# alexandrainst/coral

Hardware: AMD Instinct MI355X
Metric: audio-seconds/sec (CTC finetune step: fwd+bwd+allreduce+clip+AdamW), wav2vec2-large, 10 s utterances (higher is better)
Workload: dtype bf16; 1 GPU; wav2vec2-large (XLS-R shape d=1920 L=48 ffn=7680) CTC finetune, 8 x 10 s per GPU, SpecAugment on, activation_dropout 0.1, layerdrop 0 (multi-GPU rule), fp32 master + AdamW + clip 1.0; global_batch=8, frames_per_utt=499, parallelism=dp1

## Files before the change

### coral_amd/_lib.py

```python

from __future__ import annotations

import ctypes as C
import os
from pathlib import Path

_HERE = Path(__file__).resolve().parent
LIB_PATH = _HERE / "libcoral_amd.so"


class CoralAmdError(RuntimeError):
    """Raised when the HIP library is missing or a call into it fails."""


class CaGemmDesc(C.Structure):

    _fields_ = [
        ("A", C.c_void_p),
        ("B", C.c_void_p),
        ("C", C.c_void_p),
        ("C2", C.c_void_p),
        ("R", C.c_void_p),
        ("bias", C.c_void_p),
        ("M", C.c_int32),
# ... 202 lines not shown
    "ca_wave_normalize": (C.c_int, [_vp, _vp, _vp, _i32, _i64, _f32, _vp]),
    "ca_frame_lengths": (C.c_int, [_vp, _i32, _i64, C.POINTER(C.c_int32), C.POINTER(C.c_int32), _i32, _vp, _vp]),
    "ca_wave_scale": (C.c_int, [_vp, _vp, _vp, _i32, _i64, _vp]),
    "ca_fir_filter": (C.c_int, [_vp, _vp, _vp, _vp, _vp, _i64, _i32, _vp, _i32, _i64, _vp]),
    "ca_mix_noise": (C.c_int, [_vp, _vp, _vp, _i64, _i64, _vp, _vp, _vp, _vp, _i32, _i64, _vp]),
    "ca_white_noise": (C.c_int, [_vp, _i64, C.c_uint64, _vp]),
    "ca_pcm_prepare": (C.c_int, [_vp, _i32, _i64, _vp, _vp, _vp, _i32, _i64, _i32, _i32, _f32, _vp]),
    "ca_resample": (C.c_int, [_vp, _i32, _i64, _vp, _vp, _i32, _vp, _vp, _i32, _i32, _i32, _vp, _i64, _vp, _i32, _vp]),
    "ca_conv0_ln_gelu_fwd": (
        C.c_int,
        [_vp, _vp, _vp, _vp, _vp, _vp, _i32, _i64, _i32, _i32, _i32, _f32, _vp],
    ),
    "ca_conv0_bwd_partial_floats": (_i64, [_i32, _i64, _i32, _i32, _i32]),
    "ca_conv0_ln_gelu_bwd": (
        C.c_int,
        [_vp] * 11 + [_i32, _i64, _i32, _i32, _i32, _f32, _vp],
    ),
    "ca_col2im_1d": (C.c_int, [_vp, _vp, _i32, _i64, _i64, _i32, _i32, _i32, _vp]),
    "ca_ctc_workspace_bytes": (_i64, [_i32, _i32, _i32]),
    "ca_ctc_loss_fwd_bwd": (
        C.c_int,
        [_vp, _vp, _vp, _vp, _vp, _vp, _vp, _i32, _i32, _i32, _i64, _i32, _i32, _i32, _vp],
    ),
    "ca_ctc_greedy_decode": (
        C.c_int,
        [_vp, _vp, _vp, _vp, _vp, _i32, _i32, _i32, _i64, _i32, _vp],
    ),
    "ca_ctc_stitch": (C.c_int, [_vp, _vp, _vp, _vp, _i32, _i32, _i32, _i64, _i32, _i32, _vp]),
    "ca_ctc_collapse_workspace_bytes": (_i64, [_i32, _i32]),
    "ca_ctc_collapse_offsets": (C.c_int, [_vp, _vp, _vp, _vp, _vp, _vp, _vp, _i64, _i32, _i32, _i32, _vp]),
    "ca_ctc_beam_workspace_bytes": (_i64, [_i32, _i32, _i32, _i32]),
    "ca_ctc_beam_decode": (C.c_int, [C.POINTER(CaCtcBeamDesc), _vp]),
    "ca_ctc_align_workspace_bytes": (_i64, [_i32, _i32, _i32]),
    "ca_ctc_align": (C.c_int, [_vp, _i64, _vp, _vp, _vp, _vp, _vp, _vp, _vp, _vp, _i64, _i32, _i32, _i32, _i32, _i32,
                               _vp]),
    "ca_edit_counts_workspace_bytes": (_i64, [_i32, _i64, _i64]),
    "ca_edit_counts": (C.c_int, [_vp, _vp, _vp, _vp, _vp, _i32, _vp, _i32, _vp, _i64, _vp]),
    "ca_beam_select_workspace_bytes": (_i64, [_i32, _i32, _i32]),
    "ca_beam_select": (C.c_int, [_vp, _i64, _vp, _vp, _i32, _i32, _i32, _vp, _vp, _vp, _vp, _i64, _vp]),
    "ca_beam_advance": (C.c_int, [C.POINTER(CaBeamDesc), _vp]),
    "ca_mask_frames": (C.c_int, [_vp, _vp, _vp, _vp, _vp, _i32, _i32, _i32, _vp]),
    "ca_regroup_pad": (C.c_int, [_vp, _vp, _i32, _i32, _i32, _i32, _i32, _vp]),
    "ca_posconv_partial_floats": (_i64, [_i32]),
    "ca_posconv_weight": (C.c_int, [_vp, _vp, _vp, _vp, _vp, _vp, _i32, _i32, _i32, _vp]),
    "ca_posconv_weight_bwd": (
        C.c_int,
# ... 96 lines not shown
```

### coral_amd/blocks.py

```python

from __future__ import annotations

import os

import torch

from . import ops
from .ops import EPI_DGELU, EPI_GELU, EPI_RESIDUAL, MNMAJOR


LN_IN_GEMM = os.environ.get("CA_DECODE_LN_FUSED", "1") != "0"


def _z(n, dev, dt=torch.bfloat16):
    return torch.zeros(n, dtype=dt, device=dev)


def zeros_on(dev):
    return lambda n, dt=torch.bfloat16: _z(n, dev, dt)


class Scratch:

    def __init__(self, M, d, f, z, Mkv=0, masks=True):
# ... 268 lines not shown
        if defer is None:
            ops.colsum(sc.du, f, M, f, g32, sc.part, out_off=o(self.fc1 + ".bias"))
        wg.append(dict(dY=sc.du, X=sv["x"], M=f, N=d, K=M, lda=f, ldb=d, c_off=o(self.fc1 + ".weight"), accumulate=acc,
                       sq=sq.get("fc1"),
                       **(dict(bias_off=o(self.fc1 + ".bias"), part=sc.part, cs_off=self.cs_fc1) if defer is not None else {})))
        if defer is not None:
            defer.extend(wg)
        else:
            ops.wgrad_gemm_group(wg, g32)
        if du8 is not None and du8["ready"][0]:
            ops.gemm_fp8(du8["buf"], fb[0], sc.dx, a_scale=du8["inv"], b_scale=du8["inv_w"], M=M, N=d, K=f, lda=f, ldb=f, ldc=d,
                         b_off=du8["w_off"])
        else:
            ops.gemm(sc.du, p16, sc.dx, M=M, N=d, K=f, lda=f, b_layout=MNMAJOR, ldb=d, ldc=d, b_off=o(self.fc1 + ".weight"))
        _ln_bwd(st, self.ln, sc.dx, sv, dh, dhin, sc, M, d, ln_part, pending, xdrop)


def wgrad_stream(engine):
    if os.environ.get("CA_WGRAD_STREAM", "1") == "0":
        return None
    if engine._wstream is None:
        engine._wstream = ops.side_stream(engine.device, "wgrad", int(os.environ.get("CA_WGRAD_PRIO", "0")))
    return engine._wstream


def norm_plan(store, matrices, device):
    if not matrices:
        return None
    off, soff, mats = 0, {}, []
    for l, key, name, M, N in matrices:
        soff[(l, key)] = off
        off += ops.sumsq_slots(M, N)
        mats.append((store.off(name), M * N))
    chunks, pos = [], 0
    for a, n in sorted(mats) + [(store.numel, 0)]:
        while pos < a:
            m = min(65536, a - pos)
            chunks.append((pos, m))
            pos += m
        pos = max(pos, a + n)
    return dict(slots=torch.zeros(off, dtype=torch.float32, device=device), nslots=off, slot_off=soff,
                chunks=torch.tensor(chunks, dtype=torch.int64, device=device), nchunks=len(chunks),
                partial=torch.zeros(max(4096, len(chunks)), dtype=torch.float32, device=device))


def encoder_backward(blocks, svs, keep, B, T, ring, scs, bias_ws, ln_parts, *, gm, acc, plan, names, side, wgrad_early,
                     matrix_range, done, below=None, mring=None, epilogue=None, rows=None):
    main = torch.cuda.current_stream()
    M = B * T if rows is None else rows[1]
    kw_rows = {} if rows is None else dict(rows=rows)

    def on_side(fn):
        if side is None:
            return fn()
        ev = torch.cuda.Event()
        ev.record(main)
        side.wait_event(ev)
        with torch.cuda.stream(side):
            return fn()

    wdone, it = {}, 0
    for l in reversed(range(len(blocks))):
        if not keep[l]:
            if not acc:
                lo, hi = matrix_range(l)
                ops.clear_ranges(gm, ((lo, hi - lo),))
                if plan is not None:
                    a0 = plan["slot_off"][(l, "qkv")]
                    ops.clear_f32(plan["slots"], plan["slot_off"].get((l + 1, "qkv"), plan["nslots"]) - a0, off=a0)
            done(names[l])
# ... 16 lines not shown

        def wgrads():
            fused[0] = ops.wgrad_gemm_group(wg, gm, colsum_ws=bw, colsum_ld=nb, Gb=g32)

        ff.backward(ring[i0], ring[i1], sv_f, sc, M, defer=wg, acc=acc, sq=sq, ln_part=lnp[0], pending=second, **kw_f)
        sa.backward(ring[i1], ring[i2], sv_a, sc, B, T, defer=wg, acc=acc, sq=sq, ln_part=lnp[1], pending=second,
                    deferred=(lambda: on_side(wgrads)) if wgrad_early else None, **kw_a, **kw_rows)

        def finish():
            if not wgrad_early:
                wgrads()
            if fused[0]:
                second.append((bw, ops.COLSUM_PARTS, nb, nb, g32[st.off(sa.qbias):], True))
            ops.reduce_rows_multi(second)
            if epilogue is not None:
                epilogue(l)
            if side is not None:
                wdone[it] = torch.cuda.Event()
                wdone[it].record(side)
            done(names[l])

        on_side(finish)
        it += 1
    if side is not None:
        main.wait_stream(side)
    k = (2 * it) % 6
    return ring[k], (mring[k] if mring is not None else None), ring[(k + 1) % 6]
```

### coral_amd/csrc/ctc.hip

```cpp
#include "common.h"

#define NEG_INF (-__builtin_inff())

__device__ __forceinline__ float log_add3(float a, float b, float c) {
  const float m = fmaxf(a, fmaxf(b, c));
  if (m == NEG_INF) return NEG_INF;
  return m + __logf(__expf(a - m) + __expf(b - m) + __expf(c - m));
}
__device__ __forceinline__ float log_add2(float a, float b) {
  const float m = fmaxf(a, b);
  if (m == NEG_INF) return NEG_INF;
  return m + __logf(__expf(a - m) + __expf(b - m));
}

struct CtcWs {
  float* lp;
  float* alpha;
  float* beta;
};

__device__ __host__ inline int64_t align256(int64_t x) { return (x + 255) & ~(int64_t)255; }

extern "C" int64_t ca_ctc_workspace_bytes(int32_t B, int32_t T, int32_t Lmax) {
  const int64_t S = 2 * (int64_t)Lmax + 1;
// ... 197 lines not shown
    }
  }
  if (tid == 0) {
    float nll;
    if (Tin <= 0) {
      nll = __builtin_inff();
    } else {
      const int lastrow = (Tin - 1) & 1;
      const float l1 = rowa[lastrow][S - 1];
      const float l2 = S >= 2 ? rowa[lastrow][S - 2] : NEG_INF;
      nll = -log_add2(l1, l2);
    }
    sh_nll = nll;
  }
  __syncthreads();
  float nll = sh_nll;
  const bool infeasible = !(nll < __builtin_inff());
  if (tid == 0) {
    nll_out[b] = (infeasible && zero_inf) ? 0.f : nll;
    raw_nll[b] = nll;
  }
}

__global__ __launch_bounds__(512) void ctc_grad_kernel(const int32_t* __restrict__ labels,
                                                       const int32_t* __restrict__ in_len,
                                                       const float* __restrict__ raw_nll, float* __restrict__ grad,
                                                       const float* __restrict__ gscale, const float* __restrict__ lp,
                                                       const float* __restrict__ alpha, const float* __restrict__ beta,
                                                       int T, int V, int64_t ldv, int Lmax, int Smax, int blank) {
  __shared__ int ext[CTC_MAXS];
  __shared__ float vm[8][256], vs[8][256];
  __shared__ int sh_L;
  const int b = blockIdx.y;
  const int tid = threadIdx.x;
  const int lane = tid & 63, wave = tid >> 6;
  if (tid == 0) {
    int L = 0;
    for (int i = 0; i < Lmax; ++i) {
      const int c = labels[(int64_t)b * Lmax + i];
      if (c >= 0) {
        ext[2 * L] = blank;
        ext[2 * L + 1] = c;
        ++L;
      }
    }
    ext[2 * L] = blank;
    sh_L = L;
  }
  __syncthreads();
  const int S = 2 * sh_L + 1;
  int Tin = in_len ? in_len[b] : T;
  if (Tin > T) Tin = T;
  if (Tin < 0) Tin = 0;
  const float nll = raw_nll[b];
  const bool infeasible = !(nll < __builtin_inff());
  const float gs = gscale ? gscale[b] : 1.f;
  const int t = blockIdx.x * 8 + wave;
  if (t >= T) return;
  float* g = grad + ((int64_t)b * T + t) * ldv;
  if (t >= Tin || infeasible) {
    for (int v = lane; v < (int)ldv; v += 64) g[v] = 0.f;
    return;
  }
  float* vmax = vm[wave];
  float* vsum = vs[wave];
  for (int v = lane; v < V; v += 64) {
    vmax[v] = NEG_INF;
    vsum[v] = 0.f;
  }
  const float* at = alpha + ((int64_t)b * T + t) * Smax;
// ... 33 lines not shown
  CA_CHECK_ARG(B > 0 && T > 0 && V > 0 && V <= 256 && ldv >= V && Lmax >= 0,
               "ca_ctc_loss_fwd_bwd: bad shape (V must be <= 256)");
  CA_CHECK_ARG(2 * Lmax + 1 <= CTC_MAXS, "ca_ctc_loss_fwd_bwd: Lmax %d too long (max %d)", Lmax,
               (CTC_MAXS - 1) / 2);
  CA_CHECK_ARG(blank >= 0 && blank < V, "ca_ctc_loss_fwd_bwd: bad blank");
  const int Smax = 2 * Lmax + 1;
  char* w = (char*)ws;
  float* lp = (float*)w;
  w += align256((int64_t)B * T * 256 * 4);
  float* alpha = (float*)w;
  w += align256((int64_t)B * T * Smax * 4);
  float* beta = (float*)w;
  w += align256((int64_t)B * T * Smax * 4);
  float* raw_nll = (float*)w;
  hipStream_t s = (hipStream_t)stream;
  const int64_t frames = (int64_t)B * T;
  hipLaunchKernelGGL(ctc_logsoftmax_kernel, dim3((unsigned)((frames + 3) / 4)), dim3(256), 0, s, logits, lp, frames, V,
                     ldv);
  const size_t lp_bytes = (size_t)T * V * sizeof(float);
  const int lp_in_lds = lp_bytes <= 120 * 1024 ? 1 : 0;
  static bool attr = false;
  if (!attr) {
    hipFuncSetAttribute((const void*)ctc_kernel, hipFuncAttributeMaxDynamicSharedMemorySize, 120 * 1024);
    attr = true;
  }
  hipLaunchKernelGGL(ctc_kernel, dim3(B), dim3(512), lp_in_lds ? lp_bytes : 0, s, labels, in_len, nll, raw_nll, lp, alpha,
                     beta, T, V, Lmax, Smax, blank, zero_infinity, lp_in_lds);
  if (grad)
    hipLaunchKernelGGL(ctc_grad_kernel, dim3((unsigned)((T + 7) / 8), B), dim3(512), 0, s, labels, in_len, raw_nll, grad,
                       gscale, lp, alpha, beta, T, V, ldv, Lmax, Smax, blank);
  CA_CHECK_LAUNCH("ca_ctc_loss_fwd_bwd");
  return CA_OK;
}

__global__ __launch_bounds__(1024) void ctc_greedy_kernel(const float* __restrict__ logits,
                                                          const int32_t* __restrict__ in_len,
                                                          int32_t* __restrict__ raw,
                                                          int32_t* __restrict__ ids,
                                                          int32_t* __restrict__ out_len, int T,
                                                          int V, int64_t ldv, int blank) {
  extern __shared__ int sh[];
  const int b = blockIdx.x;
  const float* lg = logits + (int64_t)b * T * ldv;
  int32_t* rb = raw + (int64_t)b * T;
  int32_t* ib = ids + (int64_t)b * T;
  int Tin = in_len ? in_len[b] : T;
  if (Tin > T) Tin = T;
  for (int t = threadIdx.x; t < T; t += 1024) {
    const float* l = lg + (int64_t)t * ldv;
    float best = l[0];
// ... 46 lines not shown
```

### coral_amd/stem_blocks.py

```python

from __future__ import annotations

import torch

from . import ops
from .blocks import layernorm_bwd
from .ops import EPI_GELU_RESIDUAL, EPI_RESIDUAL, MNMAJOR

F32 = torch.float32


class ConvScratch:

    def __init__(self, z, B, wgrad, dgrad, part):
        nw = max(c.Co * c.k * c.Ci for c in wgrad)
        self.dwr_part, self.dwr = z(B * nw, F32), z(nw, F32)
        self.dcol = z(max(B * c.T * c.k * c.Ci for c in dgrad))
        self.part = part


class StridedConvBlock:

    def __init__(self, store, weight: str, bias: str, Ci: int, Co: int, k: int, stride: int, rows_in=None, rows_out=None,
                 y_off: int = 0):
        self.st, self.Ci, self.Co, self.k, self.stride, self.y_off = store, Ci, Co, k, stride, y_off
        self.w_off, self.b_off = store.off(weight), store.off(bias)
        self.wr = torch.zeros(Co * k * Ci, dtype=torch.bfloat16, device=store.device)
        if rows_in is not None:
            self.set_rows(rows_in, rows_out)

    def set_rows(self, rows_in: int, rows_out=None):
        self.rows_in = rows_in
        self.T = (rows_in - self.k) // self.stride + 1
        self.rows_out = self.T if rows_out is None else rows_out
        assert self.y_off + self.T <= self.rows_out

    def refresh(self):
        ops.conv_weight_reorder(self.st.p32, self.wr, self.Co, self.Ci, self.k, w_off=self.w_off)

    def forward(self, x, y, B, **epilogue):
        Ci, Co, k = self.Ci, self.Co, self.k
        ops.gemm(x, self.wr, y, c_off=self.y_off * Co, M=self.T, N=Co, K=k * Ci, lda=self.stride * Ci, ldb=k * Ci, ldc=Co,
                 bias=self.st.p32, bias_off=self.b_off, batch2=B, sA=(0, self.rows_in * Ci), sC=(0, self.rows_out * Co),
                 **epilogue)

    def backward(self, dy, x, B, sc: ConvScratch, dx=None):
        Ci, Co, k, T = self.Ci, self.Co, self.k, self.T
        g32, nw = self.st.g32, Co * k * Ci
        clips, rows = (1, B * T) if self.rows_out == T else (B, T)
        for b in range(clips):
            ops.colsum(dy, Co, rows, Co, g32, sc.part, x_off=(b * self.rows_out + self.y_off) * Co, out_off=self.b_off)
        ops.gemm(dy, x, sc.dwr_part, M=Co, N=k * Ci, K=T, a_layout=MNMAJOR, lda=Co, a_off=self.y_off * Co, b_layout=MNMAJOR,
                 ldb=self.stride * Ci, ldc=k * Ci, out_f32=True, batch2=B, sA=(0, self.rows_out * Co),
                 sB=(0, self.rows_in * Ci), sC=(0, nw))
        ops.reduce_rows(sc.dwr_part, B, nw, nw, sc.dwr)
        ops.conv_weight_grad_reorder(sc.dwr, g32, Co, Ci, k, dw_off=self.w_off)
        if dx is not None:
            assert self.rows_out == T, "the data gradient reads dy as one [B * T, Co] matrix"
            ops.gemm(dy, self.wr, sc.dcol, M=B * T, N=k * Ci, K=Co, lda=Co, b_layout=MNMAJOR, ldb=k * Ci, ldc=k * Ci)
            ops.col2im_1d(sc.dcol, dx, B, T, self.rows_in, Ci, k, self.stride)


class ConvFeatureEncoder:

    def __init__(self, store, prefix: str, conv_dim, conv_kernel, conv_stride, eps: float, f32: bool):
        assert conv_dim[0] == 512 and conv_kernel[0] == 10, "layer-0 kernel expects C=512,k=10"
        self.st, self.eps, self.f32 = store, eps, f32
        self.dims, self.k0, self.stride0 = tuple(conv_dim), conv_kernel[0], conv_stride[0]
        names = [[f"{prefix}{i}.{n}" for n in ("conv.weight", "conv.bias", "layer_norm.weight", "layer_norm.bias")]
                 for i in range(len(conv_dim))]
        self.p = [[store.view(n) for n in ns] for ns in names]
        self.g = [[store.view(n, "g32") for n in ns] for ns in names]
        self.convs = [None] + [StridedConvBlock(store, names[i][0], names[i][1], conv_dim[i - 1], conv_dim[i], conv_kernel[i],
                                                conv_stride[i]) for i in range(1, len(conv_dim))]

    def refresh(self):
        for c in self.convs[1:]:
            c.refresh()

    def alloc(self, B, Ts, z, part):
        n = [B * T * C for T, C in zip(Ts, self.dims)]
        bf, cdt = torch.bfloat16, F32 if self.f32 else torch.bfloat16
        for i, c in enumerate(self.convs[1:], 1):
            c.set_rows(Ts[i - 1])
        return dict(Ts=Ts, a=[z(m, dt=bf) for m in n[:-1]] + [z(n[-1], dt=cdt)], y=[None] + [z(m, dt=cdt) for m in n[1:]],
                    cstats=[None] + [z(B * T * 2, dt=F32) for T in Ts[1:]], dconv=[z(m) for m in n], dy=z(max(n[1:])),
                    sc=ConvScratch(z, B, self.convs[1:], self.convs[1:], part))

    def forward(self, x, sv, B, N):
        a, y, Ts = sv["a"], sv["y"], sv["Ts"]
        ops.conv0_fwd(x, *self.p[0], a[0], B, N, self.dims[0], self.k0, self.stride0, self.eps)
        for i, c in enumerate(self.convs[1:], 1):
            c.set_rows(Ts[i - 1])
            c.forward(a[i - 1], y[i], B)
            ops.layernorm_fwd(y[i], self.p[i][2], self.p[i][3], a[i], sv["cstats"][i], B * Ts[i], c.Co, self.eps, act=1)
        return a[-1]

    def backward(self, x, sv, B, N):
        dconv, dy, sc, Ts = sv["dconv"], sv["dy"], sv["sc"], sv["Ts"]
        for i in range(len(self.convs) - 1, 0, -1):
            c, (_, _, gamma, beta), (_, _, dgamma, dbeta) = self.convs[i], self.p[i], self.g[i]
            ops.layernorm_bwd(dconv[i], sv["y"][i], gamma, beta, sv["cstats"][i], None, dy, dgamma, dbeta, sc.part,
                              B * Ts[i], c.Co, act=1)
            c.backward(dy, sv["a"][i - 1], B, sc, dx=dconv[i - 1])
        ops.conv0_bwd(x, *self.p[0], dconv[0], *self.g[0], sc.part, B, N, self.dims[0], self.k0, self.stride0, self.eps)


class FeatureProjection:

    def __init__(self, store, prefix: str, C: int, d: int, eps: float):
        self.st, self.C, self.d, self.eps = store, C, d, eps
        ln = prefix + "layer_norm."
        self.gamma, self.beta = store.view(ln + "weight"), store.view(ln + "bias")
        self.dgamma, self.dbeta = store.view(ln + "weight", "g32"), store.view(ln + "bias", "g32")
        self.w_off, self.b_off = store.off(prefix + "projection.weight"), store.off(prefix + "projection.bias")

    def alloc(self, M, z):
        return dict(xln=z(M * self.C), st=z(M * 2, dt=F32))

    def forward(self, x, h0, sv, M, drop=(0.0, 0)):
        st, C, d = self.st, self.C, self.d
        ops.layernorm_fwd(x, self.gamma, self.beta, sv["xln"], sv["st"], M, C, self.eps)
        ops.gemm(sv["xln"], st.p16, h0, M=M, N=d, K=C, lda=C, ldb=C, ldc=d, b_off=self.w_off, bias=st.p32, bias_off=self.b_off)
        if drop[0] > 0:
            ops.dropout(h0, h0, M * d, *drop)

    def backward(self, dh0, x, dxln, dx, sv, M, part, drop=(0.0, 0)):
        st, C, d = self.st, self.C, self.d
        if drop[0] > 0:
            ops.dropout(dh0, dh0, M * d, *drop)
        ops.colsum(dh0, d, M, d, st.g32, part, out_off=self.b_off)
        ops.gemm(dh0, sv["xln"], st.g32, M=d, N=C, K=M, a_layout=MNMAJOR, lda=d, b_layout=MNMAJOR, ldb=C, ldc=C,
                 c_off=self.w_off, out_f32=True, accumulate=True)
        ops.gemm(dh0, st.p16, dxln, M=M, N=C, K=d, lda=d, b_layout=MNMAJOR, ldb=C, ldc=C, b_off=self.w_off)
        ops.layernorm_bwd(dxln, x, self.gamma, None, sv["st"], None, dx, self.dgamma, self.dbeta, part, M, C)


class PosConvEmbed:

    def __init__(self, store, prefix: str, d: int, G: int, K: int):
        self.st, self.d, self.G, self.K, self.Cg = store, d, G, K, d // G
        dev = store.device
        self.wf = torch.zeros(d * K * self.Cg, dtype=torch.bfloat16, device=dev)
        self.wb = torch.zeros(d * K * self.Cg, dtype=torch.bfloat16, device=dev)
        self.norm = torch.zeros(K, dtype=F32, device=dev)
        self.partial = torch.zeros(ops.posconv_partial_floats(K), dtype=F32, device=dev)
        w = prefix + "parametrizations.weight."
        self.v, self.g = store.view(w + "original1"), store.view(w + "original0")
        self.dv, self.dg = store.view(w + "original1", "g32"), store.view(w + "original0", "g32")
        self.b_off = store.off(prefix + "bias")

    def refresh(self):
        ops.posconv_weight(self.v, self.g, self.wf, self.wb, self.norm, self.partial, self.d, self.Cg, self.K)

    def alloc(self, B, T, z):
        n = B * self.G * (T + self.K) * self.Cg + 8 * self.Cg
        return dict(xg=z(n), pc_pre=z(B * T * self.d), dxg=z(n), dwf=z(self.d * self.K * self.Cg, dt=F32))

    def _conv(self, T, Tpad):
        G, K, Cg, d = self.G, self.K, self.Cg, self.d
        return dict(M=T, N=Cg, K=K * Cg, lda=Cg, ldb=K * Cg, ldc=d, ldr=d, batch2=G, sA=(G * Tpad * Cg, Tpad * Cg),
                    sB=(0, Cg * K * Cg), sC=(T * d, Cg), sR=(T * d, Cg))

    def forward(self, h0, h, sv, B, T):
        st, G, K, Cg = self.st, self.G, self.K, self.Cg
        ops.regroup_pad(h0, sv["xg"], B, T, G, Cg, K // 2)
        ops.gemm(sv["xg"], self.wf, sv["pc_pre"], C2=h, R=h0, bias=st.p32, bias_off=self.b_off, epilogue=EPI_GELU_RESIDUAL,
                 batch1=B, sBias=(0, Cg), **self._conv(T, T + K))

    def backward(self, dh, dpc, dh0, sv, B, T, part):
        st, d, G, K, Cg = self.st, self.d, self.G, self.K, self.Cg
        M, Tpad = B * T, T + K
        ops.dgelu_mul(dh, sv["pc_pre"], dpc, M * d)
        ops.colsum(dpc, d, M, d, st.g32, part, out_off=self.b_off)
        ops.gemm(dpc, sv["xg"], sv["dwf"], M=Cg, N=K * Cg, K=M, a_layout=MNMAJOR, lda=d, b_layout=MNMAJOR, ldb=Cg, b_kseg=T,
                 b_kseg_stride=G * Tpad * Cg, ldc=K * Cg, batch2=G, sA=(0, Cg), sB=(0, Tpad * Cg), sC=(0, Cg * K * Cg),
                 out_f32=True)
        ops.posconv_weight_bwd(sv["dwf"], self.v, self.g, self.norm, self.dv, self.dg, self.partial, d, Cg, K)
        ops.regroup_pad(dpc, sv["dxg"], B, T, G, Cg, K // 2)
        ops.gemm(sv["dxg"], self.wb, dh0, a_off=Cg, epilogue=EPI_RESIDUAL, R=dh, batch1=B, **self._conv(T, Tpad))


class LMHead:

    def __init__(self, store, ln: str, weight: str, bias: str | None, d: int, V: int, eps: float):
        self.st, self.d, self.V, self.Vp, self.eps = store, d, V, (V + 7) // 8 * 8, eps
        self.gamma, self.beta = store.view(ln + ".weight"), store.view(ln + ".bias")
        self.dgamma, self.dbeta = store.view(ln + ".weight", "g32"), store.view(ln + ".bias", "g32")
        self.w_off = store.off(weight)
        self.b_off = store.off(bias) if bias is not None else None

    def alloc(self, M, z, train=True):
        return dict(hf=z(M * self.d), st=z(M * 2, dt=F32) if train else None)

    def forward(self, h, sv, M, logits=None, last_of=None, drop=(0.0, 0)):
        d, hf = self.d, sv["hf"]
        ops.layernorm_fwd(h, self.gamma, self.beta, hf, sv["st"], M, d, self.eps)
        if drop[0] > 0:
            ops.dropout(hf, hf, M * d, *drop)
        if last_of is None:
            return self.project(hf, M, logits)
# ... 23 lines not shown
```

### coral_amd/wav2vec2.py

```python

from __future__ import annotations

import math
import os
from dataclasses import dataclass

import torch

from . import ops
from .blocks import FFNBlock, Scratch, SelfAttnBlock, encoder_backward, wgrad_stream
from .engine import Engine
from .staging import PinnedStager
from .stem_blocks import ConvFeatureEncoder, FeatureProjection, LMHead, PosConvEmbed


@dataclass
class Wav2Vec2Shape:

    hidden_size: int = 1024
    num_hidden_layers: int = 24
    num_attention_heads: int = 16
    intermediate_size: int = 4096
    conv_dim: tuple = (512,) * 7
    conv_kernel: tuple = (10, 3, 3, 3, 3, 2, 2)
    conv_stride: tuple = (5, 2, 2, 2, 2, 2, 2)
    num_conv_pos_embeddings: int = 128
    num_conv_pos_embedding_groups: int = 16
    vocab_size: int = 46
    pad_token_id: int = 45
    layer_norm_eps: float = 1e-5
    ctc_loss_reduction: str = "sum"
    ctc_zero_infinity: bool = True
    activation_dropout: float = 0.0
# ... 314 lines not shown
        for k, st in zip(self.s.conv_kernel, self.s.conv_stride):
            n = torch.div(n - k, st, rounding_mode="floor") + 1
        return n

    def _workspace(self, B: int, N: int):
        key = (B, N)
        if self._ws_key == key:
            return self._ws
        s, dev = self.s, self.device
        d, f = s.hidden_size, s.intermediate_size
        L = s.num_hidden_layers
        Ts = self.conv_lengths(N)
        T = Ts[-1]
        M = B * T
        bf, f32 = torch.bfloat16, torch.float32

        def build(z):
            w = {"B": B, "N": N, "Ts": Ts, "T": T, "M": M}
            pf = max(
                ops.layernorm_bwd_partial_floats(B * Ts[1], 512), ops.layernorm_bwd_partial_floats(M, d),
                ops.colsum_partial_floats(M, max(f, 3 * d)), ops.colsum_partial_floats(B * Ts[1], 512),
                ops.conv0_bwd_partial_floats(B, N, s.conv_dim[0], s.conv_kernel[0], s.conv_stride[0]), 4096)
            w["partial"] = z(pf, dt=f32)
            w["fe"] = self.feature_encoder.alloc(B, Ts, z, w["partial"])
            w["fp"] = self.feature_projection.alloc(M, z)
            w["h0"] = z(M * d)
            w["pc"] = self.pos_conv.alloc(B, T, z)
            w["h"] = [z(M * d) for _ in range(L + 1)]
            w["hpk"] = z(M * d)
            w["h1"] = [z(M * d) for _ in range(L)]
            w["sv"] = [(sa.alloc(B, T, z), ff.alloc(M, z)) for sa, ff in self.blocks]
            w["head"] = self.head.alloc(M, z)
            Vp = w["Vp"] = self.head.Vp
            w["logits"] = z(M * Vp, dt=f32)
            w["dlogits"] = z(M * Vp, dt=f32)
            w["dlogits16"] = z(M * Vp)
            w["dlogits16p"] = z(M * Vp)
            w["nll"] = z(B, dt=f32)
            w["dA"] = z(M * d)
            w["ring"] = [z(M * d) for _ in range(6)]
            w["mring"] = [z(M * d) for _ in range(6)] if s.hidden_dropout > 0 else None
            w["scs"] = [Scratch(M, d, f, z, masks=False) for _ in range(2)]
            w["bias_ws"] = [z(ops.COLSUM_PARTS * (5 * d + f), dt=f32) for _ in range(2)]
            w["ln_partial"] = [[z(ops.layernorm_bwd_partial_floats(M, d), dt=f32) for _ in range(2)] for _ in range(2)]
            return w

# ... 123 lines not shown
            ops.wave_scale(dl, self._scale_scalar(loss_scale), dl, 1, M * Vp)
        ops.cast_f32_bf16(dl, w["dlogits16"], M * Vp)
        d16 = w["dlogits16"]
        rows, hs = sv["rows"], sv["hs"]
        Me = M if rows is None else rows[1]
        if rows is not None:
            ops.pack_rows(d16, w["dlogits16p"], rows[0], B, T, Vp)
            d16 = w["dlogits16p"]
        tr = sv["training"]

        def branch_site(j):
            below = [k for k in range(j) if keep[k]]
            if not below and rows is not None:
                return 0.0, 0
            return self.dropout_site("ffn_out", below[-1], tr) if below else self.dropout_site("pos_conv", training=tr)

        ring, mring = w["ring"], w["mring"]
        drop = branch_site(L)
        self.head.backward(d16, hs[L], w["dA"], ring[0], w["head"], Me, part, freeze=self.freeze_base,
                           drop=self.dropout_site("final", training=tr), xdrop=(*drop, mring[0]) if drop[0] > 0 else None)
        done("head")
        if self.freeze_base:
            return
        dh, dhm, dpc = encoder_backward(
            self.blocks, w["sv"], keep, B, T, ring, w["scs"], w["bias_ws"], w["ln_partial"], gm=gm, acc=lacc,
            plan=self.norm_plan(), names=[f"layer{l}" for l in range(L)], side=wgrad_stream(self), wgrad_early=True,
            matrix_range=lambda l: self.shard_ranges()[f"layer{l}"], done=done, below=branch_site, mring=mring,
            **({} if rows is None else dict(rows=rows)))
        dg = dhm if branch_site(0)[0] > 0 else dh
        if rows is not None:
            dg = next(r for r in ring if r is not dh and r is not dpc)
            ops.unpack_rows(dh, dg, rows[0], B, T, d)
            pc = self.dropout_site("pos_conv", training=tr)
            if pc[0] > 0:
                ops.dropout(dg, dg, M * d, *pc)
        dh0 = w["dA"]
        self.pos_conv.backward(dg, dpc, dh0, w["pc"], B, T, part)
        if sv["tm"] is not None:
            ops.colsum(dh0, d, M, d, st.g32, part, rowmask=sv["tm"], out_off=st.off("wav2vec2.masked_spec_embed"))
        ops.mask_frames(dh0, sv["tm"], sv["fm"], self.zero_embed, flen, B, T, d)
        fe = w["fe"]
        self.feature_projection.backward(dh0, fe["a"][-1], fe["dy"], fe["dconv"][-1], w["fp"], M, part,
                                         self.dropout_site("feat_proj", training=tr))
        self.feature_encoder.backward(x, fe, B, N)
        done("front")

    def _scale_scalar(self, v: float) -> torch.Tensor:
        cache = self.__dict__.setdefault("_scalars", {})
        t = cache.get(v)
        if t is None:
            if len(cache) > 64:
                cache.clear()
            t = cache[v] = torch.full((1,), float(v), dtype=torch.float32, device=self.device)
        return t

    def greedy_decode(self, logits_full: torch.Tensor | None = None, in_len=None):
        sv = self._saved
        w = sv["w"]
        B, T, V, Vp = sv["B"], w["T"], self.s.vocab_size, w["Vp"]
        dev = self.device
        raw = torch.empty(B, T, dtype=torch.int32, device=dev)
        ids = torch.empty(B, T, dtype=torch.int32, device=dev)
        olen = torch.empty(B, dtype=torch.int32, device=dev)
        ops.ctc_greedy_decode(w["logits"], in_len, raw, ids, olen, B, T, V, Vp, self.s.pad_token_id)
        ids_c, olen_c = ids.cpu(), olen.cpu()
        return [ids_c[b, :int(olen_c[b])].tolist() for b in range(B)], raw

# ... 78 lines not shown
```

### include/coral_amd.h

```cpp
#ifndef CORAL_AMD_H
#define CORAL_AMD_H

#include <stdint.h>

#ifdef __cplusplus
extern "C" {
#endif

#define CA_OK 0
#define CA_ERR_ARG (-1)
#define CA_ERR_LAUNCH (-2)
#define CA_ERR_UNSUPPORTED (-3)

int ca_version(void);
const char* ca_last_error(void);
int ca_device_count(void);

#define CA_KMAJOR 0
#define CA_MNMAJOR 1

#define CA_EPI_NONE 0
#define CA_EPI_GELU 1
#define CA_EPI_RESIDUAL 2
#define CA_EPI_DGELU 3
// ... 50 lines not shown
int ca_fp8_amax_rotate(uint32_t* amax_next, float* scale, float* inv_scale, int32_t count, float margin, void* stream);
int ca_dropout_rows_fp8(const void* x, void* y, void* q_fp8, float* row_scale, int64_t rows, int32_t C, float p,
                        uint64_t seed, void* stream);
int ca_quantize_fp8_transposed(const void* x_bf16, int32_t rows, int32_t cols, void* q_fp8_t, const float* scale,
                               void* stream);
#define CA_FP8_GROUP_MAX 8
typedef struct CaFp8RefreshTask {
  const void* x_bf16;
  void* q_fp8;
  void* q_fp8_t;
  const float* scale;
  uint32_t* amax_next;
  int32_t rows, cols;
} CaFp8RefreshTask;
int ca_fp8_refresh_group(const CaFp8RefreshTask* tasks, int32_t count, void* stream);
int ca_gemm_bf16_group(const CaGemmDesc* descs, int32_t count, void* stream);

int ca_prof_begin(void);
int ca_prof_end(double* ms, int64_t* count, double* flops);

int ca_gemm_force_kernel(int which);
int ca_gemm_debug_general_epilogue(int on);
int ca_debug_cu_hog(int32_t blocks, int32_t threads, int32_t lds_bytes, double ms, void* stream);

int ca_gemm_set_compute_cus(int n);

int ca_layernorm_fwd(const void* x, const float* gamma, const float* beta, void* y,
                     float* stats, int64_t rows, int32_t C, float eps, int32_t act,
                     void* stream);
int ca_layernorm_fwd_ex(const void* x, const float* gamma, const float* beta, void* y,
                        float* stats, int64_t rows, int32_t C, float eps, int32_t act,
                        int32_t x_f32, int32_t y_f32, void* stream);
int ca_layernorm_fwd_fp8(const void* x, const float* gamma, const float* beta, void* y, void* q_fp8,
                         float* row_scale, float* stats, int64_t rows, int32_t C, float eps, void* stream);
int64_t ca_layernorm_bwd_partial_floats(int64_t rows, int32_t C);
int ca_layernorm_bwd(const void* dy, const void* x, const float* gamma, const float* beta,
                     const float* stats, const void* dres, void* dx, float* dgamma,
                     float* dbeta, float* partial, int64_t rows, int32_t C, int32_t act,
                     void* stream);

int ca_layernorm_bwd_ex(const void* dy, const void* x, const float* gamma, const float* beta,
                        const float* stats, const void* dres, void* dx, float* dgamma,
                        float* dbeta, float* partial, int64_t rows, int32_t C, int32_t act,
                        int32_t x_f32, void* stream);

int ca_layernorm_bwd_dropout(const void* dy, const void* x, const float* gamma, const float* beta,
// ... 383 lines not shown
```

Measured before the change: 1127 audio-seconds/sec.

## Overlap stem weight-grads on side stream and add wave-level CTC kernel

Moves the weight-gradient work of the positional conv, feature projection and conv feature encoder onto the wgrad side stream through a LeafLane helper. The encoder backward no longer joins the side stream before the stem, so its trailing weight-gradients can overlap with the front-end backward, with per-layer events and a double-buffered dy to keep data ordering correct. It also adds a single-wave CTC alpha/beta kernel that runs forward and backward in separate blocks, keeps four states per lane and passes neighbours through DPP, and parallelizes label extension with ballot. The costs are a separate partial buffer and more cross-stream event traffic.

```diff
diff --git a/coral_amd/_lib.py b/coral_amd/_lib.py
--- a/coral_amd/_lib.py
+++ b/coral_amd/_lib.py
@@ -248,6 +248,7 @@
         C.c_int,
         [_vp, _vp, _vp, _vp, _vp, _vp, _vp, _i32, _i32, _i32, _i64, _i32, _i32, _i32, _vp],
     ),
+    "ca_ctc_set_form": (C.c_int, [C.c_int]),
     "ca_ctc_greedy_decode": (
         C.c_int,
         [_vp, _vp, _vp, _vp, _vp, _i32, _i32, _i32, _i64, _i32, _vp],
diff --git a/coral_amd/blocks.py b/coral_amd/blocks.py
--- a/coral_amd/blocks.py
+++ b/coral_amd/blocks.py
@@ -314,6 +314,33 @@
     if engine._wstream is None:
         engine._wstream = ops.side_stream(engine.device, "wgrad", int(os.environ.get("CA_WGRAD_PRIO", "0")))
     return engine._wstream
+
+
+class LeafLane:
+
+    def __init__(self, side, part):
+        self.side, self.part, self.main = side, part, torch.cuda.current_stream()
+
+    def run(self, fn):
+        if self.side is None:
+            fn()
+            return None
+        ev = torch.cuda.Event()
+        ev.record(self.main)
+        self.side.wait_event(ev)
+        with torch.cuda.stream(self.side):
+            fn()
+            end = torch.cuda.Event()
+            end.record(self.side)
+        return end
+
+    def wait(self, ev):
+        if ev is not None:
+            self.main.wait_event(ev)
+
+
+def tail_overlap():
+    return os.environ.get("CA_TAIL_OVERLAP", "1") != "0"
 
 
 def norm_plan(store, matrices, device):
@@ -337,7 +364,7 @@
 
 
 def encoder_backward(blocks, svs, keep, B, T, ring, scs, bias_ws, ln_parts, *, gm, acc, plan, names, side, wgrad_early,
-                     matrix_range, done, below=None, mring=None, epilogue=None, rows=None):
+                     matrix_range, done, below=None, mring=None, epilogue=None, rows=None, join=True):
     main = torch.cuda.current_stream()
     M = B * T if rows is None else rows[1]
     kw_rows = {} if rows is None else dict(rows=rows)
@@ -400,7 +427,7 @@
 
         on_side(finish)
         it += 1
-    if side is not None:
+    if side is not None and join:
         main.wait_stream(side)
     k = (2 * it) % 6
     return ring[k], (mring[k] if mring is not None else None), ring[(k + 1) % 6]
diff --git a/coral_amd/csrc/ctc.hip b/coral_amd/csrc/ctc.hip
--- a/coral_amd/csrc/ctc.hip
+++ b/coral_amd/csrc/ctc.hip
@@ -243,6 +243,147 @@
   }
 }
 
+static int g_ctc_form = 0;
+extern "C" int ca_ctc_set_form(int form) {
+  CA_CHECK_ARG(form == 0 || form == 1, "ca_ctc_set_form: 0 (by label width) or 1 (block kernel)");
+  g_ctc_form = form;
+  return CA_OK;
+}
+
+#define CTC_WAVE_LMAX 127
+
+__device__ __forceinline__ int ctc_extend_wave(const int32_t* __restrict__ lab, int Lmax, int blank, int* ext, int lane) {
+  int L = 0;
+  for (int base = 0; base < Lmax; base += 64) {
+    const int i = base + lane;
+    const int c = i < Lmax ? lab[i] : -1;
+    const unsigned long long m = __ballot(c >= 0);
+    if (c >= 0) {
+      const int p = L + __popcll(m & ((1ull << lane) - 1ull));
+      ext[2 * p] = blank;
+      ext[2 * p + 1] = c;
+    }
+    L += __popcll(m);
+  }
+  if (lane == 0) ext[2 * L] = blank;
+  return L;
+}
+
+__device__ __forceinline__ float ctc_lane_up(float inject, float v) {
+  return __builtin_bit_cast(float, __builtin_amdgcn_update_dpp(__builtin_bit_cast(int, inject), __builtin_bit_cast(int, v),
+                                                                0x138, 0xf, 0xf, false));
+}
+__device__ __forceinline__ float ctc_lane_down(float inject, float v) {
+  return __builtin_bit_cast(float, __builtin_amdgcn_update_dpp(__builtin_bit_cast(int, inject), __builtin_bit_cast(int, v),
+                                                                0x130, 0xf, 0xf, false));
+}
+
+template <bool LDS_LP>
+__global__ __launch_bounds__(256) void ctc_wave_kernel(const int32_t* __restrict__ labels,
+                                                       const int32_t* __restrict__ in_len, float* __restrict__ nll_out,
+                                                       float* __restrict__ raw_nll, const float* __restrict__ lp,
+                                                       float* __restrict__ alpha, float* __restrict__ beta, int T, int V,
+                                                       int Lmax, int Smax, int blank, int zero_inf) {
+  __shared__ int ext[2 * CTC_WAVE_LMAX + 2];
+  __shared__ float last[2 * CTC_WAVE_LMAX + 2];
+  __shared__ int sh_L;
+  extern __shared__ float lds_lp[];
+  const int b = blockIdx.x;
+  const bool fwd = blockIdx.y == 0;
+  const int tid = threadIdx.x;
+  const int lane = tid & 63;
+  const float* lpb = lp + (int64_t)b * T * V;
+  int Tin = in_len ? in_len[b] : T;
+  if (Tin > T) Tin = T;
+  if (Tin < 0) Tin = 0;
+  if (LDS_LP)
+    for (int i = tid; i < Tin * V; i += 256) lds_lp[i] = lpb[i];
+  if (tid < 64) {
+    const int n = ctc_extend_wave(labels + (int64_t)b * Lmax, Lmax, blank, ext, lane);
+    if (lane == 0) sh_L = n;
+  }
+  __syncthreads();
+  if (tid >= 64) return;
+  const int S = 2 * sh_L + 1;
+  if (Tin <= 0) {
+    if (fwd && lane == 0) {
+      nll_out[b] = zero_inf ? 0.f : __builtin_inff();
+      raw_nll[b] = __builtin_inff();
+    }
+    return;
+  }
+  float* tab = (fwd ? alpha : beta) + (int64_t)b * T * Smax + 4 * lane;
+  int c[4];
+  bool skip[4], valid[4];
+  float a[4];
+#pragma unroll
+  for (int j = 0; j < 4; ++j) {
+    const int s = 4 * lane + j;
+    valid[j] = s < S;
+    c[j] = valid[j] ? ext[s] : blank;
+    const int s2 = fwd ? s - 2 : s + 2;
+    skip[j] = valid[j] && s2 >= 0 && s2 < S && c[j] != blank && ext[s2] != c[j];
+  }
+  auto lpv = [&](int tt, int cc) -> float { return LDS_LP ? lds_lp[tt * V + cc] : lpb[(int64_t)tt * V + cc]; };
+  const int t0 = fwd ? 0 : Tin - 1;
+#pragma unroll
+  for (int j = 0; j < 4; ++j) {
+    const int s = 4 * lane + j;
+    const bool init = fwd ? (s == 0 || s == 1) : (s == S - 1 || s == S - 2);
+    a[j] = (valid[j] && init) ? lpv(t0, c[j]) : NEG_INF;
+    if (valid[j]) tab[(int64_t)t0 * Smax + j] = a[j];
+  }
+  float nx[4];
+  if (Tin > 1) {
+#pragma unroll
+    for (int j = 0; j < 4; ++j) nx[j] = lpv(fwd ? 1 : Tin - 2, c[j]);
+  }
+  for (int step = 1; step < Tin; ++step) {
+    const int tt = fwd ? step : Tin - 1 - step;
+    const float n1 = fwd ? ctc_lane_up(NEG_INF, a[3]) : ctc_lane_down(NEG_INF, a[0]);
+    const float n2 = fwd ? ctc_lane_up(NEG_INF, a[2]) : ctc_lane_down(NEG_INF, a[1]);
+    float cur[4];
+#pragma unroll
+    for (int j = 0; j < 4; ++j) cur[j] = nx[j];
+    if (step + 1 < Tin) {
+#pragma unroll
+      for (int j = 0; j < 4; ++j) nx[j] = lpv(fwd ? step + 1 : Tin - 2 - step, c[j]);
+    }
+    float na[4];
+    if (fwd) {
+      na[0] = log_add3(a[0], n1, skip[0] ? n2 : NEG_INF);
+      na[1] = log_add3(a[1], a[0], skip[1] ? n1 : NEG_INF);
+      na[2] = log_add3(a[2], a[1], skip[2] ? a[0] : NEG_INF);
+      na[3] = log_add3(a[3], a[2], skip[3] ? a[1] : NEG_INF);
+    } else {
+      na[3] = log_add3(a[3], n1, skip[3] ? n2 : NEG_INF);
+      na[2] = log_add3(a[2], a[3], skip[2] ? n1 : NEG_INF);
+      na[1] = log_add3(a[1], a[2], skip[1] ? a[3] : NEG_INF);
+      na[0] = log_add3(a[0], a[1], skip[0] ? a[2] : NEG_INF);
+    }
+#pragma unroll
+    for (int j = 0; j < 4; ++j) {
+      a[j] = valid[j] ? na[j] + cur[j] : NEG_INF;
+      if (valid[j]) tab[(int64_t)tt * Smax + j] = a[j];
+    }
+  }
+  if (!fwd) return;
+#pragma unroll
+  for (int j = 0; j < 4; ++j)
+    if (valid[j]) last[4 * lane + j] = a[j];
+  __builtin_amdgcn_fence(__ATOMIC_RELEASE, "wavefront");
+  __builtin_amdgcn_wave_barrier();
+  __builtin_amdgcn_fence(__ATOMIC_ACQUIRE, "wavefront");
+  if (lane == 0) {
+    const float l1 = last[S - 1];
+    const float l2 = S >= 2 ? last[S - 2] : NEG_INF;
+    const float nll = -log_add2(l1, l2);
+    const bool infeasible = !(nll < __builtin_inff());
+    nll_out[b] = (infeasible && zero_inf) ? 0.f : nll;
+    raw_nll[b] = nll;
+  }
+}
+
 __global__ __launch_bounds__(512) void ctc_grad_kernel(const int32_t* __restrict__ labels,
                                                        const int32_t* __restrict__ in_len,
                                                        const float* __restrict__ raw_nll, float* __restrict__ grad,
@@ -255,18 +396,9 @@
   const int b = blockIdx.y;
   const int tid = threadIdx.x;
   const int lane = tid & 63, wave = tid >> 6;
-  if (tid == 0) {
-    int L = 0;
-    for (int i = 0; i < Lmax; ++i) {
-      const int c = labels[(int64_t)b * Lmax + i];
-      if (c >= 0) {
-        ext[2 * L] = blank;
-        ext[2 * L + 1] = c;
-        ++L;
-      }
-    }
-    ext[2 * L] = blank;
-    sh_L = L;
+  if (tid < 64) {
+    const int n = ctc_extend_wave(labels + (int64_t)b * Lmax, Lmax, blank, ext, lane);
+    if (lane == 0) sh_L = n;
   }
   __syncthreads();
   const int S = 2 * sh_L + 1;
@@ -346,10 +478,20 @@
   static bool attr = false;
   if (!attr) {
     hipFuncSetAttribute((const void*)ctc_kernel, hipFuncAttributeMaxDynamicSharedMemorySize, 120 * 1024);
+    hipFuncSetAttribute((const void*)ctc_wave_kernel<true>, hipFuncAttributeMaxDynamicSharedMemorySize, 120 * 1024);
     attr = true;
   }
-  hipLaunchKernelGGL(ctc_kernel, dim3(B), dim3(512), lp_in_lds ? lp_bytes : 0, s, labels, in_len, nll, raw_nll, lp, alpha,
-                     beta, T, V, Lmax, Smax, blank, zero_infinity, lp_in_lds);
+  if (g_ctc_form == 0 && Lmax <= CTC_WAVE_LMAX) {
+    if (lp_in_lds)
+      hipLaunchKernelGGL(ctc_wave_kernel<true>, dim3(B, 2), dim3(256), lp_bytes, s, labels, in_len, nll, raw_nll, lp, alpha,
+                         beta, T, V, Lmax, Smax, blank, zero_infinity);
+    else
+      hipLaunchKernelGGL(ctc_wave_kernel<false>, dim3(B, 2), dim3(256), 0, s, labels, in_len, nll, raw_nll, lp, alpha, beta,
+                         T, V, Lmax, Smax, blank, zero_infinity);
+  } else {
+    hipLaunchKernelGGL(ctc_kernel, dim3(B), dim3(512), lp_in_lds ? lp_bytes : 0, s, labels, in_len, nll, raw_nll, lp, alpha,
+                       beta, T, V, Lmax, Smax, blank, zero_infinity, lp_in_lds);
+  }
   if (grad)
     hipLaunchKernelGGL(ctc_grad_kernel, dim3((unsigned)((T + 7) / 8), B), dim3(512), 0, s, labels, in_len, raw_nll, grad,
                        gscale, lp, alpha, beta, T, V, ldv, Lmax, Smax, blank);
diff --git a/coral_amd/stem_blocks.py b/coral_amd/stem_blocks.py
--- a/coral_amd/stem_blocks.py
+++ b/coral_amd/stem_blocks.py
@@ -44,21 +44,27 @@
                  bias=self.st.p32, bias_off=self.b_off, batch2=B, sA=(0, self.rows_in * Ci), sC=(0, self.rows_out * Co),
                  **epilogue)
 
-    def backward(self, dy, x, B, sc: ConvScratch, dx=None):
+    def backward(self, dy, x, B, sc: ConvScratch, dx=None, lane=None):
         Ci, Co, k, T = self.Ci, self.Co, self.k, self.T
         g32, nw = self.st.g32, Co * k * Ci
-        clips, rows = (1, B * T) if self.rows_out == T else (B, T)
-        for b in range(clips):
-            ops.colsum(dy, Co, rows, Co, g32, sc.part, x_off=(b * self.rows_out + self.y_off) * Co, out_off=self.b_off)
-        ops.gemm(dy, x, sc.dwr_part, M=Co, N=k * Ci, K=T, a_layout=MNMAJOR, lda=Co, a_off=self.y_off * Co, b_layout=MNMAJOR,
-                 ldb=self.stride * Ci, ldc=k * Ci, out_f32=True, batch2=B, sA=(0, self.rows_out * Co),
-                 sB=(0, self.rows_in * Ci), sC=(0, nw))
-        ops.reduce_rows(sc.dwr_part, B, nw, nw, sc.dwr)
-        ops.conv_weight_grad_reorder(sc.dwr, g32, Co, Ci, k, dw_off=self.w_off)
+        part = sc.part if lane is None else lane.part
+
+        def wgrad():
+            clips, rows = (1, B * T) if self.rows_out == T else (B, T)
+            for b in range(clips):
+                ops.colsum(dy, Co, rows, Co, g32, part, x_off=(b * self.rows_out + self.y_off) * Co, out_off=self.b_off)
+            ops.gemm(dy, x, sc.dwr_part, M=Co, N=k * Ci, K=T, a_layout=MNMAJOR, lda=Co, a_off=self.y_off * Co, b_layout=MNMAJOR,
+                     ldb=self.stride * Ci, ldc=k * Ci, out_f32=True, batch2=B, sA=(0, self.rows_out * Co),
+                     sB=(0, self.rows_in * Ci), sC=(0, nw))
+            ops.reduce_rows(sc.dwr_part, B, nw, nw, sc.dwr)
+            ops.conv_weight_grad_reorder(sc.dwr, g32, Co, Ci, k, dw_off=self.w_off)
+
+        ev = lane.run(wgrad) if lane is not None else wgrad()
         if dx is not None:
             assert self.rows_out == T, "the data gradient reads dy as one [B * T, Co] matrix"
             ops.gemm(dy, self.wr, sc.dcol, M=B * T, N=k * Ci, K=Co, lda=Co, b_layout=MNMAJOR, ldb=k * Ci, ldc=k * Ci)
             ops.col2im_1d(sc.dcol, dx, B, T, self.rows_in, Ci, k, self.stride)
+        return ev
 
 
 class ConvFeatureEncoder:
@@ -85,7 +91,7 @@
             c.set_rows(Ts[i - 1])
         return dict(Ts=Ts, a=[z(m, dt=bf) for m in n[:-1]] + [z(n[-1], dt=cdt)], y=[None] + [z(m, dt=cdt) for m in n[1:]],
                     cstats=[None] + [z(B * T * 2, dt=F32) for T in Ts[1:]], dconv=[z(m) for m in n], dy=z(max(n[1:])),
-                    sc=ConvScratch(z, B, self.convs[1:], self.convs[1:], part))
+                    dy2=z(max(n[1:])), sc=ConvScratch(z, B, self.convs[1:], self.convs[1:], part))
 
     def forward(self, x, sv, B, N):
         a, y, Ts = sv["a"], sv["y"], sv["Ts"]
@@ -96,13 +102,17 @@
             ops.layernorm_fwd(y[i], self.p[i][2], self.p[i][3], a[i], sv["cstats"][i], B * Ts[i], c.Co, self.eps, act=1)
         return a[-1]
 
-    def backward(self, x, sv, B, N):
-        dconv, dy, sc, Ts = sv["dconv"], sv["dy"], sv["sc"], sv["Ts"]
+    def backward(self, x, sv, B, N, lane=None):
+        dconv, dys, sc, Ts = sv["dconv"], (sv["dy"], sv["dy2"]), sv["sc"], sv["Ts"]
+        evs = {}
         for i in range(len(self.convs) - 1, 0, -1):
             c, (_, _, gamma, beta), (_, _, dgamma, dbeta) = self.convs[i], self.p[i], self.g[i]
+            dy = dys[i & 1]
+            if lane is not None:
+                lane.wait(evs.pop(i + 2, None))
             ops.layernorm_bwd(dconv[i], sv["y"][i], gamma, beta, sv["cstats"][i], None, dy, dgamma, dbeta, sc.part,
                               B * Ts[i], c.Co, act=1)
-            c.backward(dy, sv["a"][i - 1], B, sc, dx=dconv[i - 1])
+            evs[i] = c.backward(dy, sv["a"][i - 1], B, sc, dx=dconv[i - 1], lane=lane)
         ops.conv0_bwd(x, *self.p[0], dconv[0], *self.g[0], sc.part, B, N, self.dims[0], self.k0, self.stride0, self.eps)
 
 
@@ -125,13 +135,16 @@
         if drop[0] > 0:
             ops.dropout(h0, h0, M * d, *drop)
 
-    def backward(self, dh0, x, dxln, dx, sv, M, part, drop=(0.0, 0)):
+    def backward(self, dh0, x, dxln, dx, sv, M, part, drop=(0.0, 0), lane=None):
         st, C, d = self.st, self.C, self.d
         if drop[0] > 0:
             ops.dropout(dh0, dh0, M * d, *drop)
-        ops.colsum(dh0, d, M, d, st.g32, part, out_off=self.b_off)
-        ops.gemm(dh0, sv["xln"], st.g32, M=d, N=C, K=M, a_layout=MNMAJOR, lda=d, b_layout=MNMAJOR, ldb=C, ldc=C,
-                 c_off=self.w_off, out_f32=True, accumulate=True)
+        def wgrad():
+            ops.colsum(dh0, d, M, d, st.g32, part if lane is None else lane.part, out_off=self.b_off)
+            ops.gemm(dh0, sv["xln"], st.g32, M=d, N=C, K=M, a_layout=MNMAJOR, lda=d, b_layout=MNMAJOR, ldb=C, ldc=C,
+                     c_off=self.w_off, out_f32=True, accumulate=True)
+
+        lane.run(wgrad) if lane is not None else wgrad()
         ops.gemm(dh0, st.p16, dxln, M=M, N=C, K=d, lda=d, b_layout=MNMAJOR, ldb=C, ldc=C, b_off=self.w_off)
         ops.layernorm_bwd(dxln, x, self.gamma, None, sv["st"], None, dx, self.dgamma, self.dbeta, part, M, C)
 
@@ -168,15 +181,18 @@
         ops.gemm(sv["xg"], self.wf, sv["pc_pre"], C2=h, R=h0, bias=st.p32, bias_off=self.b_off, epilogue=EPI_GELU_RESIDUAL,
                  batch1=B, sBias=(0, Cg), **self._conv(T, T + K))
 
-    def backward(self, dh, dpc, dh0, sv, B, T, part):
+    def backward(self, dh, dpc, dh0, sv, B, T, part, lane=None):
         st, d, G, K, Cg = self.st, self.d, self.G, self.K, self.Cg
         M, Tpad = B * T, T + K
         ops.dgelu_mul(dh, sv["pc_pre"], dpc, M * d)
-        ops.colsum(dpc, d, M, d, st.g32, part, out_off=self.b_off)
-        ops.gemm(dpc, sv["xg"], sv["dwf"], M=Cg, N=K * Cg, K=M, a_layout=MNMAJOR, lda=d, b_layout=MNMAJOR, ldb=Cg, b_kseg=T,
-                 b_kseg_stride=G * Tpad * Cg, ldc=K * Cg, batch2=G, sA=(0, Cg), sB=(0, Tpad * Cg), sC=(0, Cg * K * Cg),
-                 out_f32=True)
-        ops.posconv_weight_bwd(sv["dwf"], self.v, self.g, self.norm, self.dv, self.dg, self.partial, d, Cg, K)
+        def wgrad():
+            ops.colsum(dpc, d, M, d, st.g32, part if lane is None else lane.part, out_off=self.b_off)
+            ops.gemm(dpc, sv["xg"], sv["dwf"], M=Cg, N=K * Cg, K=M, a_layout=MNMAJOR, lda=d, b_layout=MNMAJOR, ldb=Cg,
+                     b_kseg=T, b_kseg_stride=G * Tpad * Cg, ldc=K * Cg, batch2=G, sA=(0, Cg), sB=(0, Tpad * Cg),
+                     sC=(0, Cg * K * Cg), out_f32=True)
+            ops.posconv_weight_bwd(sv["dwf"], self.v, self.g, self.norm, self.dv, self.dg, self.partial, d, Cg, K)
+
+        lane.run(wgrad) if lane is not None else wgrad()
         ops.regroup_pad(dpc, sv["dxg"], B, T, G, Cg, K // 2)
         ops.gemm(sv["dxg"], self.wb, dh0, a_off=Cg, epilogue=EPI_RESIDUAL, R=dh, batch1=B, **self._conv(T, Tpad))
 
diff --git a/coral_amd/wav2vec2.py b/coral_amd/wav2vec2.py
--- a/coral_amd/wav2vec2.py
+++ b/coral_amd/wav2vec2.py
@@ -8,7 +8,7 @@
 import torch
 
 from . import ops
-from .blocks import FFNBlock, Scratch, SelfAttnBlock, encoder_backward, wgrad_stream
+from .blocks import FFNBlock, LeafLane, Scratch, SelfAttnBlock, encoder_backward, tail_overlap, wgrad_stream
 from .engine import Engine
 from .staging import PinnedStager
 from .stem_blocks import ConvFeatureEncoder, FeatureProjection, LMHead, PosConvEmbed
@@ -369,6 +369,7 @@
                 ops.colsum_partial_floats(M, max(f, 3 * d)), ops.colsum_partial_floats(B * Ts[1], 512),
                 ops.conv0_bwd_partial_floats(B, N, s.conv_dim[0], s.conv_kernel[0], s.conv_stride[0]), 4096)
             w["partial"] = z(pf, dt=f32)
+            w["partial_leaf"] = z(pf, dt=f32)
             w["fe"] = self.feature_encoder.alloc(B, Ts, z, w["partial"])
             w["fp"] = self.feature_projection.alloc(M, z)
             w["h0"] = z(M * d)
@@ -538,11 +539,14 @@
         done("head")
         if self.freeze_base:
             return
+        side = wgrad_stream(self)
+        overlap = tail_overlap() and side is not None
         dh, dhm, dpc = encoder_backward(
             self.blocks, w["sv"], keep, B, T, ring, w["scs"], w["bias_ws"], w["ln_partial"], gm=gm, acc=lacc,
-            plan=self.norm_plan(), names=[f"layer{l}" for l in range(L)], side=wgrad_stream(self), wgrad_early=True,
+            plan=self.norm_plan(), names=[f"layer{l}" for l in range(L)], side=side, wgrad_early=True,
             matrix_range=lambda l: self.shard_ranges()[f"layer{l}"], done=done, below=branch_site, mring=mring,
-            **({} if rows is None else dict(rows=rows)))
+            join=not overlap or rows is not None, **({} if rows is None else dict(rows=rows)))
+        lane = LeafLane(side, w["partial_leaf"]) if overlap else None
         dg = dhm if branch_site(0)[0] > 0 else dh
         if rows is not None:
             dg = next(r for r in ring if r is not dh and r is not dpc)
@@ -551,14 +555,16 @@
             if pc[0] > 0:
                 ops.dropout(dg, dg, M * d, *pc)
         dh0 = w["dA"]
-        self.pos_conv.backward(dg, dpc, dh0, w["pc"], B, T, part)
+        self.pos_conv.backward(dg, dpc, dh0, w["pc"], B, T, part, lane=lane)
         if sv["tm"] is not None:
             ops.colsum(dh0, d, M, d, st.g32, part, rowmask=sv["tm"], out_off=st.off("wav2vec2.masked_spec_embed"))
         ops.mask_frames(dh0, sv["tm"], sv["fm"], self.zero_embed, flen, B, T, d)
         fe = w["fe"]
         self.feature_projection.backward(dh0, fe["a"][-1], fe["dy"], fe["dconv"][-1], w["fp"], M, part,
-                                         self.dropout_site("feat_proj", training=tr))
-        self.feature_encoder.backward(x, fe, B, N)
+                                         self.dropout_site("feat_proj", training=tr), lane=lane)
+        self.feature_encoder.backward(x, fe, B, N, lane=lane)
+        if overlap:
+            torch.cuda.current_stream().wait_stream(side)
         done("front")
 
     def _scale_scalar(self, v: float) -> torch.Tensor:
diff --git a/include/coral_amd.h b/include/coral_amd.h
--- a/include/coral_amd.h
+++ b/include/coral_amd.h
@@ -96,6 +96,7 @@
 int ca_gemm_force_kernel(int which);
 int ca_gemm_debug_general_epilogue(int on);
 int ca_debug_cu_hog(int32_t blocks, int32_t threads, int32_t lds_bytes, double ms, void* stream);
+int ca_ctc_set_form(int form);
 
 int ca_gemm_set_compute_cus(int n);
 
```

New measurement: 1135 audio-seconds/sec (median of 6 runs). Within noise of the previous version (+0.7%).
